# rdesc/autorally

Hardware: AMD Instinct MI355X
Metric: trajectory rollouts/s per MPPI solve (higher is better)
Workload: dtype f32

## Files before the change

### autorally_amd/csrc/abi_solve.hip

```cpp
#include "abi_internal.hpp"

using namespace mppi;
using namespace mppi_abi;

namespace mppi_abi {

std::mutex g_batch_mu;
hipStream_t g_batch_stream[64] = {};
hipStream_t batch_stream(int device)
{
  if (device < 0 || device >= 64) return nullptr;
  std::lock_guard<std::mutex> lk(g_batch_mu);
  if (!g_batch_stream[device] &&
      hipStreamCreateWithFlags(&g_batch_stream[device], hipStreamNonBlocking) != hipSuccess)
    g_batch_stream[device] = nullptr;
  return g_batch_stream[device];
}

void fill_cost_args(const mppi_handle *h, CostArgs &c)
{
  const mppi_cost_params &p = h->cost;
  c.desired_speed = p.desired_speed;
  c.speed_coeff = p.speed_coeff;
  c.track_coeff = p.track_coeff;
// ... 388 lines not shown
  if (rc) return rc;
  const bool timed = h->timing && (h->timing_count++ % (unsigned)h->timing_every) == 0;
  const bool explicit_noise = h->explicit_iters > 0;
  const size_t slot_sz = (size_t)K * T * 2;
  h->seq = next_seq(h);
  for (int it = 0; it < iters; it++) {
    Events *ev = timed ? &h->ev[it] : nullptr;
    if (ev) HIPCHK(h, hipEventRecord(ev->e[0], h->stream));
    const bool inline_noise = !explicit_noise && !h->prefetch_valid && has_noise_wave(h);
    float *noise = h->d_noise + (size_t)(explicit_noise ? it : 0) * slot_sz;
    if (!explicit_noise && !inline_noise) {
      rc = acquire_noise(h, &noise);
      if (rc) return rc;
    } else if (inline_noise) {
      noise = h->d_gen[h->gen_cur];
    }
    h->v_buf = noise;
    if (ev) HIPCHK(h, hipEventRecord(ev->e[1], h->stream));
    RolloutArgs a;
    fill_rollout_args(h, state, noise, a);
    rc = tag_min_cost(h, a, h->stream);
    if (rc) return rc;
    if (inline_noise) use_inline_noise(h, a);
#ifdef MPPI_HOSTPROF
    HP(1, hp_t0);
    const auto hp_t1 = std::chrono::steady_clock::now();
#endif
    if (ev) { tl_kernel_start = ev->e[4]; tl_kernel_stop = ev->e[5]; }
    rc = launch_rollout(h, a);
    tl_kernel_start = tl_kernel_stop = nullptr;
    if (rc) return rc;
#ifdef MPPI_HOSTPROF
    HP(2, hp_t1);
    const auto hp_t2 = std::chrono::steady_clock::now();
#endif
    const bool prefetch = h->gen_async && iters == 1 && !explicit_noise && !has_noise_wave(h) && !h->prefetch_valid;
    if (prefetch) HIPCHK(h, hipEventRecord(h->ev_s1, h->stream));
    if (ev) HIPCHK(h, hipEventRecord(ev->e[2], h->stream));
    const bool last = (it == iters - 1);
    const bool want_slid = last && wants_slid_copy(h);
    next_tail_epoch(h);
    HIPCHK(h, launch_solve_tail(tail_launch(h, noise, last), h->stream));
    if (last) h->slid_valid = want_slid;
    if (h->capture) {
      float *c = h->d_cap + (size_t)it * (2 * (size_t)T + K);
      if (!last) HIPCHK(h, hipMemcpyAsync(c, h->d_in, sizeof(float) * 2 * (size_t)T, hipMemcpyDeviceToDevice, h->stream));
      HIPCHK(h, hipMemcpyAsync(c + 2 * (size_t)T, h->d_costs, sizeof(float) * (size_t)K, hipMemcpyDeviceToDevice, h->stream));
    }
    if (prefetch) {
      h->gen_time_now = timed;
      rc = prefetch_noise(h);
      h->gen_time_now = false;
      if (rc) return rc;
    }
#ifdef MPPI_HOSTPROF
    HP(3, hp_t2);
    hp_n += 1;
    if ((long)hp_n % 2000 == 0)
      fprintf(stderr, "hostprof n=%.0f: seen->enqueue %.2f us, entry->launch %.2f, rollout launch %.2f, tail launch %.2f, poll->smoothed %.2f\n",
              hp_n, hp_acc[0] / hp_n, hp_acc[1] / hp_n, hp_acc[2] / hp_n, hp_acc[3] / hp_n, hp_acc[4] / hp_n);
#endif
    if (ev) HIPCHK(h, hipEventRecord(ev->e[3], h->stream));
  }
  h->explicit_iters = 0;
  h->pending = true;
  h->pending_timed = timed;
  h->cap_valid = h->capture;
  h->cap_explicit = explicit_noise;
  return MPPI_OK;
}


static int arm_kind(const mppi_handle *h)
{
  if (!(h->d_gate != nullptr && wants_slid_copy(h) && h->cfg.num_iters == 1 && !h->timing && !h->capture &&
        h->explicit_iters == 0 && !h->basis && h->fault_wave == 0 && h->have_nn && h->have_map && h->have_cost && !h->timed_out))
    return 0;
  const Form f = form_of(h);
  if ((form_is_row(f) || f == Form::M44 || f == Form::Lds44) && has_noise_wave(h) && !h->prefetch_valid) return 1;
  if (f == Form::Multi4Tree && h->forced == Form::Auto && !has_noise_wave(h) && h->gen_async && gen_beside_rollout(h)) return 2;
  return 0;
}

static void write_gate_payload(mppi_handle *h, const float *state)
{
  unsigned *g = gate_host(h);
  const int T = h->T;
  memcpy(g + kGateUOffset, h->U.data(), sizeof(float) * 2 * (size_t)T);
  memcpy(g + gate_hist_offset(T), h->hist.data(), sizeof(float) * 4);
  for (int r = 0; r < kGateReplicas; r++) memcpy(g + 16 * r, state, sizeof(float) * kStateDim);
}

static void write_gate_word(mppi_handle *h, unsigned word)
{
  unsigned *g = gate_host(h);
  asm volatile("" ::: "memory");
  __builtin_ia32_sfence();
  for (int r = 0; r < kGateReplicas; r++) __atomic_store_n(g + 16 * r + 7, word, __ATOMIC_RELAXED);
  __builtin_ia32_sfence();
}

static unsigned arm_ticks(double max_wait_s) { return (unsigned)(max_wait_s * 1e8); }
static std::chrono::steady_clock::time_point arm_deadline(double max_wait_s)
{
  const double open_s = 0.9 * max_wait_s - 50e-6;
  return std::chrono::steady_clock::now() + std::chrono::nanoseconds((long long)((open_s > 0.0 ? open_s : 0.0) * 1e9));
}

static void armed_args(mppi_handle *h, float *noise, RolloutArgs &a, TailLaunch &l, double max_wait_s)
{
  static const float no_state[kStateDim] = {0, 0, 0, 0, 0, 0, 0};
  fill_rollout_args(h, no_state, noise, a);
  a.costs = h->d_costs_alt;
  a.U = reinterpret_cast<const float *>(gate_dev(h)) + kGateUOffset;
  a.gate = gate_dev(h);
  a.gate_seq = h->arm_seq;
  a.gate_ticks = arm_ticks(max_wait_s);
  l = tail_launch(h, noise, true);
  l.costs = h->d_costs_alt;
  l.w = h->d_w_alt;
  l.seq = h->arm_seq;
  l.hist = reinterpret_cast<const float *>(gate_dev(h)) + gate_hist_offset(h->T);
  l.U = h->d_in;
  l.hist_out = h->d_in + 2 * h->T;
  l.slid = h->d_in_buf[1 - h->in_cur];
}

static void mark_armed(mppi_handle *h, int kind, float *vbuf, hipStream_t stream, double max_wait_s, bool publish_only)
{
  h->armed = kind;
  h->arm_in = h->in_cur;
  h->arm_vbuf = vbuf;
  h->arm_stream = stream;
  h->arm_until = arm_deadline(max_wait_s);
  h->arm_n = 0;
  h->arm_publish_only = publish_only;
  h->u_dirty = true;
  h->slid_valid = false;
}

static int arm_handle(mppi_handle *h, int kind, hipStream_t stream, double max_wait_s, bool publish_only, bool mark,
                      RolloutArgs &a, TailLaunch &l)
{
  h->arm_seq = next_seq(h);
  h->gate_blk ^= 1;
  float *noise = h->d_gen[1 - h->gen_cur];
  if (kind == 2) {
    int rc = acquire_noise(h, &noise);
    if (rc) return rc;
  }
  if (mark) HIPCHK(h, hipEventRecord(h->ev_arm, stream));
  armed_args(h, noise, a, l, max_wait_s);
  int rc = tag_min_cost(h, a, stream);
  if (rc) return rc;
  l.min_cost_tag = h->min_cost_tag;
  if (publish_only) {
    l.no_device_copy = 1;
    l.slid = nullptr;
  }
  if (kind == 1) use_inline_noise(h, a);
  next_tail_epoch(h);
  l.epoch = h->tail_epoch;
  mark_armed(h, kind, noise, stream, max_wait_s, publish_only);
  return MPPI_OK;
}

static int arm_one(mppi_handle *h, double max_wait_s, bool publish_only, bool mark)
{
  const int kind = arm_kind(h);
  if (!kind) return fail(h, MPPI_ERR_UNSUPPORTED, "this handle's form / configuration has no gated form (mppi_arm)");
  OWN(h);
  RolloutArgs a;
  TailLaunch l;
  int rc = arm_handle(h, kind, h->stream, max_wait_s, publish_only, mark, a, l);
  if (rc) return rc;
  rc = launch_rollout(h, a);
  if (rc == MPPI_OK) {
    const hipError_t e = launch_solve_tail(l, h->stream);
    if (e != hipSuccess) rc = fail(h, MPPI_ERR_HIP, "armed tail launch", e);
  }
  if (rc) (void)solve_ahead_disarm(h);
  return rc;
}

static int disarm_one(mppi_handle *h)
{
  if (!h->armed) return MPPI_OK;
  const int kind = h->armed;
  h->armed = 0;
  h->arm_n = 0;
  write_gate_word(h, h->arm_seq | kGateCancel);
  h->seq_floor = h->arm_seq;
  h->u_dirty = true;
  h->slid_valid = false;
  h->order_stream = h->arm_stream;
  if (kind == 1) {
    h->rng_cur = 1 - h->rng_cur;
    return MPPI_OK;
  }
  HIPCHK(h, ensure_device(h->cfg.device));
  h->gen_cur = 1 - h->gen_cur;
  h->rng_cur = 1 - h->rng_cur;
  HIPCHK(h, hipEventRecord(h->ev_s1, h->arm_stream));
  HIPCHK(h, hipStreamWaitEvent(h->gstream, h->ev_s1, 0));
  int rc = launch_generator(h, h->d_gen[1 - h->gen_cur]);
  if (rc) return rc;
  h->prefetch_valid = true;
  return MPPI_OK;
}

int solve_ahead_disarm(mppi_handle *h)
{
  if (!h || !h->armed) return MPPI_OK;
  if (h->arm_n > 0) {
    mppi_handle *peers[kMaxBatch];
    const int n = h->arm_n;
    for (int i = 0; i < n; i++) peers[i] = h->arm_peers[i];
    int rc = MPPI_OK;
    for (int i = 0; i < n; i++) {
      const int r = disarm_one(peers[i]);
      if (r && !rc) rc = r;
    }
    return rc;
  }
  return disarm_one(h);
}

static bool arm_usable(const mppi_handle *h)
{
  if (std::chrono::steady_clock::now() >= h->arm_until) return false;
  const volatile unsigned *words = reinterpret_cast<const volatile unsigned *>(h->h_res);
  const unsigned s1 = __atomic_load_n(words + 1, __ATOMIC_ACQUIRE), s3 = __atomic_load_n(words + 4 * (h->T + 1) + 1, __ATOMIC_ACQUIRE);
  return s1 != h->arm_seq && s3 != h->arm_seq;
}

static int open_armed(mppi_handle *h, const float *state)
{
  const int kind = h->armed;
  h->armed = 0;
  h->arm_n = 0;
  h->seq = h->arm_seq;
  write_gate_payload(h, state);
  write_gate_word(h, h->seq);
  h->order_stream = h->arm_stream;
  std::swap(h->d_costs, h->d_costs_alt);
  std::swap(h->d_w, h->d_w_alt);
  h->v_buf = h->arm_vbuf;
  if (kind == 1) h->gen_cur = h->arm_vbuf == h->d_gen[0] ? 0 : 1;
  h->in_cur = h->arm_in;
  h->d_in = h->d_in_buf[h->in_cur];
  h->u_dirty = h->arm_publish_only;
  h->slid_valid = !h->arm_publish_only;
  if (kind == 2) {
    const int rc = prefetch_noise(h);
    if (rc) {
      h->pending = true;
      h->pending_armed = true;
      return rc;
    }
  }
  h->pending = true;
  h->pending_timed = false;
  h->pending_armed = true;
  h->explicit_iters = 0;
  return MPPI_OK;
}

static bool batch_together(mppi_handle *const *hs, int n);
static int arm_together(mppi_handle *const *hs, int n, double max_wait_s)
{
  mppi_handle *h0 = hs[0];
  if (!form_is_row(form_of(h0))) return fail(h0, MPPI_ERR_UNSUPPORTED, "the batched launch of this form has no gated form");
  for (int i = 0; i < n; i++)
    if (arm_kind(hs[i]) != 1) return fail(hs[i], MPPI_ERR_UNSUPPORTED, "this handle's configuration has no gated form (mppi_arm_batch)");
  HIPCHK(h0, ensure_device(h0->cfg.device));
  if (!h0->batch_s) h0->batch_s = batch_stream(h0->cfg.device);
  const hipStream_t S = h0->batch_s;
  if (!S) return fail(h0, MPPI_ERR_HIP, "no batch stream");
  for (int i = 0; i < n; i++)
    if (int rc = hand_over(hs[i], S)) return rc;
  QuadBatchArgs qb;
  TailLaunch tl[kMaxBatch];
  qb.n = n;
  for (int i = 0; i < n; i++)
    if (int rc = arm_handle(hs[i], 1, S, max_wait_s, false, true, qb.inst[i], tl[i])) return rc;
  for (int i = 0; i < n; i++) {
    hs[i]->arm_n = n;
    for (int q = 0; q < n; q++) hs[i]->arm_peers[q] = hs[q];
  }
  for (int i = n; i < kMaxBatch; i++) qb.inst[i] = qb.inst[0];
  hipError_t e = launch_rollout_row_batch(qb, form_of(h0) == Form::RowTree, S);
  if (e == hipSuccess) e = launch_solve_tail_batch(tl, n, S);
  if (e != hipSuccess) {
    const int rc = fail(h0, MPPI_ERR_HIP, "armed batched launch", e);
    (void)solve_ahead_disarm(h0);
    return rc;
  }
  return MPPI_OK;
}

static bool batch_together(mppi_handle *const *hs, int n)
{
  const mppi_handle *h0 = hs[0];
  bool together = n >= 2 && n <= kMaxBatch;
  int waves = 0;
  for (int i = 0; i < n && together; i++) {
    const mppi_handle *h = hs[i];
    const Form f = form_of(h);
    const bool form_ok = h->basis ? (h0->basis && f == Form::Bf3)
                                  : (!h0->basis && (f == Form::Quad || form_is_row(f)) && f == form_of(h0) &&
                                     h->hidden == h0->hidden && h->n_hidden == h0->n_hidden);
    CostArgs ci, c0;
    fill_cost_args(h, ci);
    fill_cost_args(h0, c0);
    together = form_ok && ci.affine == c0.affine && ci.need_control_cost == c0.need_control_cost &&
               h->cfg.device == h0->cfg.device && h->cfg.num_iters == h0->cfg.num_iters &&
               h->K <= 4096 && !h->timing && !h->capture && !h->prefetch_valid && h->have_nn && h->have_map && h->have_cost;
    waves += h->basis ? 3 * (h->K / 64) : 4 * (h->K / kRolloutsPerWave);
  }
  return together && waves <= h0->num_simds;
}

static bool armed_as_batch(mppi_handle *const *hs, int n)
{
  for (int i = 0; i < n; i++) {
    if (!hs[i]->armed || hs[i]->arm_n != n) return false;
// ... 386 lines not shown
```

### autorally_amd/csrc/group_roles.hpp

```cpp
#pragma once

#include "mppi_device.hpp"
#include "noise_device.hpp"

namespace mppi {

constexpr int kGRing = 16;
constexpr int kGCtlChunk = 4;

template <class SH>
struct GroupRoles {
  static constexpr int kPose = SH::NW, kCost = SH::NW + 1, kCtl = SH::NW + 2, kRng = SH::NW + 3;
  static constexpr int kWaves = SH::NW + 4;
  static_assert(kWaves <= (int)(sizeof(SH::fin) / sizeof(int)), "fin[]");
  static_assert(SH::kR == 16 || SH::kR == 8, "rollouts per group");
};
template <class SH>
__device__ __forceinline__ int group_j(int slot) { return slot & (SH::kR - 1); }
template <class SH>
__device__ __forceinline__ bool group_real(int slot) { return slot < SH::kR; }

template <class SH>
__device__ __forceinline__ int group_seq_min(SH &sh)
{
// ... 1 lines not shown
#pragma unroll
  for (int w = 1; w < SH::NW; w++) m = min(m, lds_peek(lds_addr(&sh.xseq[w][0])));
  return m;
}

struct MrgHalf {
  uint32_t s0, s1, s2;
};
__device__ __forceinline__ uint32_t fold_m(uint64_t x, uint32_t C, uint32_t m)
{
  x = (x >> 32) * C + (x & 0xffffffffULL);
  x = (x >> 32) * C + (x & 0xffffffffULL);
  x = (x >> 32) * C + (x & 0xffffffffULL);
  if (x >= m) x -= m;
  return (uint32_t)x;
}
template <class SH>
__device__ __forceinline__ MrgHalf group_rng_load(const RolloutArgs &a)
{
  const int lane = threadIdx.x & 63;
  const int j = group_j<SH>((lane >> 1) & 15), c = lane & 1;
  const int k = (int)blockIdx.x * SH::kR + j;
  const int K = a.K;
  MrgHalf g{0, 0, 0};
  if (a.inline_noise != 0 && lane < 2 * kRolloutsPerWave) {
    g.s0 = a.rng_in[(3 * c) * K + k]; g.s1 = a.rng_in[(3 * c + 1) * K + k]; g.s2 = a.rng_in[(3 * c + 2) * K + k];
  }
  return g;
}
template <class SH, bool PRE = false>
__device__ __forceinline__ void group_rng_wave(const RolloutArgs &a, SH &sh, const MrgHalf pre = MrgHalf{0, 0, 0})
{
  using R = GroupRoles<SH>;
  const int lane = threadIdx.x & 63;
  const int j = group_j<SH>((lane >> 1) & 15), c = lane & 1;
  const int k = (int)blockIdx.x * SH::kR + j;
  const int K = a.K, T = a.T;
  const bool active = lane < 2 * kRolloutsPerWave;
  const bool real = lane < 2 * SH::kR;
  int budget = spin_budget_init(a.spin_budget, T, a.fault_wave == R::kRng + 1);
  if (a.inline_noise != 0) {
    const uint32_t m = c ? (uint32_t)kM2 : (uint32_t)kM1, C = c ? kC2 : kC1;
    const uint32_t A = c ? (uint32_t)kA21 : (uint32_t)kA12, Bn = c ? (uint32_t)kA23N : (uint32_t)kA13N;
    MrgHalf g{0, 0, 0};
    if constexpr (PRE) {
      g = pre;
    } else if (active) {
      g.s0 = a.rng_in[(3 * c) * K + k]; g.s1 = a.rng_in[(3 * c + 1) * K + k]; g.s2 = a.rng_in[(3 * c + 2) * K + k];
    }
    const uint32_t a_ctl = lds_addr(&sh.ctl_pub[0]);
    const uint32_t a_mypub = lds_addr(&sh.rng_pub[lane]);
    int seen = 0;
    for (int t = 0; t < T; t++) {
      float2 e = make_float2(0.5f, 0.5f);
#ifdef MPPI_DIAG_NORNG
      e = make_float2(0.25f + 0.001f * (float)t, 0.5f);
#else
#pragma unroll
      for (int d = 0; d < 2; d++) {
        const uint32_t p = fold_m((uint64_t)A * (c ? g.s2 : g.s1) + (uint64_t)Bn * (m - g.s0), C, m);
        g.s0 = g.s1; g.s1 = g.s2; g.s2 = p;
        const uint32_t p2 = (uint32_t)__builtin_amdgcn_mov_dpp((int)p, 0xB1, 0xF, 0xF, false);
        uint32_t z = (p >= p2) ? p - p2 : p + (uint32_t)kM1 - p2;
        if (z == 0) z = (uint32_t)kM1;
        const float u = (float)z * 0x1p-32f;
        if (d == 0) e.x = u; else e.y = u;
      }
#endif
      const int need = t - kGRing + 1;
      while (seen < need && --budget > 0) {
        seen = lds_peek(a_ctl);
        if (seen < need) __builtin_amdgcn_s_sleep(2);
      }
      if (active && c == 0) *reinterpret_cast<float2 *>(&sh.eps[t & (kGRing - 1)][j][0]) = e;
      lds_publish(a_mypub, t + 1);
    }
    if (real) {
      a.rng_out[(3 * c) * K + k] = g.s0; a.rng_out[(3 * c + 1) * K + k] = g.s1; a.rng_out[(3 * c + 2) * K + k] = g.s2;
    }
  }
  spin_finish(budget, lds_addr(&sh.fail[0]), lds_addr(&sh.fin[R::kRng]));
}

template <class SH>
__device__ __forceinline__ void group_control_wave(const RolloutArgs &a, SH &sh, const uint32_t a_gate_open = 0)
{
  using R = GroupRoles<SH>;
  constexpr int NSW = SH::NSW;
  static_assert(kGCtlChunk == 4 && kGRing >= 2 * kGCtlChunk, "four steps per iteration, lanes 16 q + j");
  const int lane = threadIdx.x & 63;
  const int j = group_j<SH>(lane & 15), q = lane >> 4;
  const bool real = group_real<SH>(lane & 15);
  const int k = (int)blockIdx.x * SH::kR + j;
  const int K = a.K, T = a.T;
  const bool inl = a.inline_noise != 0;
  float2 *const noise = reinterpret_cast<float2 *>(a.noise);
  const float2 *const Useq = reinterpret_cast<const float2 *>(a.U);
  const bool noise_free_k = (k == 0);
  const bool pure_noise_k = (k >= a.k99);
  const uint32_t a_cd = lds_addr(&sh.cost_done[0]);
  const uint32_t a_mypub = lds_addr(&sh.ctl_pub[lane]);
  const uint32_t a_rng = lds_addr(&sh.rng_pub[0]);
  int budget = spin_budget_init(a.spin_budget, T, a.fault_wave == R::kCtl + 1);
  const bool gated = a_gate_open != 0;
  if (gated)
    while (lds_peek(a_gate_open) == 0 && --budget > 0) __builtin_amdgcn_s_sleep(1);
  int seen_x = 0, seen_c = 0, seen_r = 0;
  for (int t0 = 0, n = 1; t0 < T; t0 += n, n = kGCtlChunk) {
    const int t = t0 + q;
    const bool live = (t < T) & (q < n);
    const int tl = live ? t : T - 1;
    float2 Ut;
    if (gated) {
      const unsigned long long ub = __hip_atomic_load(reinterpret_cast<const unsigned long long *>(Useq + tl), __ATOMIC_RELAXED, __HIP_MEMORY_SCOPE_SYSTEM);
      Ut = make_float2(__uint_as_float((unsigned)ub), __uint_as_float((unsigned)(ub >> 32)));
    } else {
      Ut = Useq[tl];
    }
    float2 e = (live && !inl) ? noise[(size_t)tl * K + k] : make_float2(0.0f, 0.0f);
    const int tm = min(t0 + n, T) - 1;
    const int need_x = (tm >= kGRing) ? (tm - kGRing) * NSW + 1 : 0;
    const int need_c = tm - kGRing + 1;
    while ((seen_x < need_x || seen_c < need_c) && --budget > 0) {
      seen_x = group_seq_min(sh);
      seen_c = lds_peek(a_cd);
      if (seen_x < need_x || seen_c < need_c) __builtin_amdgcn_s_sleep(2);
    }
    if (inl) {
      while (seen_r < tm + 1 && --budget > 0) {
        seen_r = lds_peek(a_rng);
        if (seen_r < tm + 1) __builtin_amdgcn_s_sleep(1);
      }
#ifdef MPPI_DIAG_NOBM
      e = *reinterpret_cast<const float2 *>(&sh.eps[tl & (kGRing - 1)][j][0]);
#else
      e = box_muller(*reinterpret_cast<const float2 *>(&sh.eps[tl & (kGRing - 1)][j][0]));
#endif
    }
    if (live) {
      const bool nf = noise_free_k | (t < a.opt_delay);
      const float n0 = e.x * a.nu[0], n1 = e.y * a.nu[1];
      const float du0 = nf ? 0.0f : n0, du1 = nf ? 0.0f : n1;
      float u0 = nf ? Ut.x : (pure_noise_k ? n0 : Ut.x + n0);
      float u1 = nf ? Ut.y : (pure_noise_k ? n1 : Ut.y + n1);
      if (real) noise[(size_t)t * K + k] = make_float2(u0, u1);
      u0 = clampf(u0, a.u_lo[0], a.u_hi[0]);
      u1 = clampf(u1, a.u_lo[1], a.u_hi[1]);
      const int slot = t & (kGRing - 1);
      sh.ctl_b1[slot][j] = u0;
      sh.ctl_b1[slot][kRolloutsPerWave + j] = u1;
      *reinterpret_cast<float4 *>(&sh.ctl_rec[slot][j][0]) = make_float4(u0, u1, du0, du1);
    }
    lds_publish(a_mypub, tm + 1);
  }
  spin_finish(budget, lds_addr(&sh.fail[0]), lds_addr(&sh.fin[R::kCtl]));
}

template <class SH, bool AFFINE>
__device__ __forceinline__ void group_pose_wave(const RolloutArgs &a, SH &sh)
{
  using R = GroupRoles<SH>;
  constexpr int NSW = SH::NSW;
  static_assert(SH::kR == 16, "one step per iteration: 16-rollout groups only");
  const int lane = threadIdx.x & 63;
  const int j = lane & 15;
  const int T = a.T;
  const uint32_t a_seq0 = lds_addr(&sh.xseq[0][0]);
  const uint32_t a_cd = lds_addr(&sh.cost_done[0]);
  const uint32_t a_mypub = lds_addr(&sh.pose_pub[lane]);
  float x = a.state[0], y = a.state[1], yaw = a.state[2];
  int budget = spin_budget_init(a.spin_budget, T, a.fault_wave == R::kPose + 1), seen = 0, cdone = 0;
  float tf_p = 0.0f, tb_p = 0.0f;
  for (int t = 0; t <= T; t++) {
    float tf = 0.0f, tb = 0.0f;
    if (t < T) {
      const int need = t * NSW + 1;
      while (seen < need && --budget > 0) {
        seen = SH::kRecByAll ? group_seq_min(sh) : lds_peek(a_seq0);
        if (seen < need) __builtin_amdgcn_s_sleep(1);
      }
      const float4 r0 = *reinterpret_cast<const float4 *>(&sh.rec[t & (kGRing - 1)][j][0]);
      float spsi, cpsi;
#ifdef MPPI_DIAG_NOPOSE
      spsi = 0.0f; cpsi = 1.0f; tf = x; tb = y;
#else
      sincos_fast(yaw, spsi, cpsi);
      const float st[3] = {x, y, yaw};
      track_fetch<AFFINE>(a.cost, st, cpsi, spsi, tf, tb);
#endif
      const float sd0 = fmaf(cpsi, r0.y, -(spsi * r0.z));
      const float sd1 = fmaf(spsi, r0.y, cpsi * r0.z);
      const float sd2 = a.negate_yaw_der ? -r0.w : r0.w;
      x = fmaf(sd0, a.dt, x);
      y = fmaf(sd1, a.dt, y);
      yaw = fmaf(sd2, a.dt, yaw);
    }
    if (t > 0) {
      while (cdone < t - kGRing && --budget > 0) cdone = lds_peek(a_cd);
      if (lane < kRolloutsPerWave) *reinterpret_cast<float2 *>(&sh.tex[(t - 1) & (kGRing - 1)][lane][0]) = make_float2(tf_p, tb_p);
      lds_publish(a_mypub, t);
    }
    tf_p = tf; tb_p = tb;
  }
  spin_finish(budget, lds_addr(&sh.fail[0]), lds_addr(&sh.fin[R::kPose]));
}

template <int Q>
__device__ __forceinline__ float quad_bc(float v)
{
  return __int_as_float(__builtin_amdgcn_mov_dpp(__float_as_int(v), Q * 0x55, 0xF, 0xF, false));
}
__device__ __forceinline__ void quad_chain(float v, float d, float dt, int q, float &vq, float &v_out)
{
  const float v1 = fmaf(quad_bc<0>(d), dt, v);
  const float v2 = fmaf(quad_bc<1>(d), dt, v1);
  const float v3 = fmaf(quad_bc<2>(d), dt, v2);
  v_out = fmaf(quad_bc<3>(d), dt, v3);
  const float lo = (q == 0) ? v : v1, hi = (q == 2) ? v2 : v3;
  vq = (q < 2) ? lo : hi;
}
template <class SH, bool AFFINE>
__device__ __forceinline__ void group_pose_wave4(const RolloutArgs &a, SH &sh, const float x0, const float y0, const float yaw0,
                                                 const int budget_cut = 0);
template <class SH, bool AFFINE>
__device__ __forceinline__ void group_pose_wave4(const RolloutArgs &a, SH &sh)
{
  group_pose_wave4<SH, AFFINE>(a, sh, a.state[0], a.state[1], a.state[2]);
}
template <class SH, bool AFFINE>
__device__ __forceinline__ void group_pose_wave4(const RolloutArgs &a, SH &sh, const float x0, const float y0, const float yaw0,
                                                 const int budget_cut)
{
  using R = GroupRoles<SH>;
  constexpr int NSW = SH::NSW;
  static_assert(kRolloutsPerWave == 16 && kGRing >= 8, "lane = 4 j + q");
  const int lane = threadIdx.x & 63;
// ... 160 lines not shown
```

### autorally_amd/csrc/mppi_device.hpp

```cpp
#pragma once

#include <hip/hip_runtime.h>
#include <stdint.h>

namespace mppi {

constexpr int kStateDim = 7;
constexpr int kControlDim = 2;
constexpr int kNetIn = 6;
constexpr int kNetOut = 4;
constexpr int kRolloutsPerWave = 16;

struct CostArgs {
  float desired_speed, speed_coeff, track_coeff, max_slip_ang, slip_penalty, track_slop;
  float crash_coeff, steering_coeff, throttle_coeff, boundary_threshold;
  float crash_cost_discounted;
  int l1_cost;
  float r_c1[3], r_c2[3], trs[3];
  int affine;
  int need_control_cost;
  int map_w, map_h;
  const float *map;
};

struct RolloutArgs {
  float state[kStateDim];
  const float *U;
  float *noise;
  float *costs;
  const float *wpack;
  const double *inv_t;
  const uint32_t *rng_in;
  uint32_t *rng_out;
  int inline_noise;
  int K, T, opt_delay, k99;
  float nu[2], u_lo[2], u_hi[2], dt;
  int negate_yaw_der;
  int spin_budget, fault_wave;
  const unsigned *gate;
  unsigned gate_seq;
  unsigned gate_ticks;
  unsigned long long *min_cost;
  unsigned min_cost_tag;
  CostArgs cost;
};
constexpr int kGateReplicas = 8;
constexpr int kGateUOffset = 16 * kGateReplicas;
inline int gate_hist_offset(int T) { return kGateUOffset + 2 * T; }
inline size_t gate_block_floats(int T) { return (size_t)gate_hist_offset(T) + 4; }
constexpr unsigned kGateCancel = 0x80000000u;

constexpr int kMinCostLines = 8, kMinCostStride = 16;
__device__ __forceinline__ unsigned cost_order_bits(float x)
{
  const unsigned b = __float_as_uint(x);
  return b ^ ((b >> 31) ? 0xFFFFFFFFu : 0x80000000u);
}
__device__ __forceinline__ float cost_from_order_bits(unsigned o)
{
  return __uint_as_float(o ^ ((o >> 31) ? 0x80000000u : 0xFFFFFFFFu));
}
template <int CTRL>
__device__ __forceinline__ float wave_dpp(float v)
{
  return __int_as_float(__builtin_amdgcn_update_dpp(0, __float_as_int(v), CTRL, 0xF, 0xF, true));
}
template <bool MIN>
__device__ __forceinline__ float wave_reduce(float v)
{
#define MPPI_RED(A, B) (MIN ? fminf((A), (B)) : (A) + (B))
  v = MPPI_RED(v, wave_dpp<0xB1>(v));
  v = MPPI_RED(v, wave_dpp<0x4E>(v));
  v = MPPI_RED(v, wave_dpp<0x141>(v));
  v = MPPI_RED(v, wave_dpp<0x140>(v));
  const auto x = __builtin_amdgcn_permlane16_swap(__float_as_uint(v), __float_as_uint(v), false, false);
  v = MPPI_RED(__uint_as_float(x[0]), __uint_as_float(x[1]));
  const auto y = __builtin_amdgcn_permlane32_swap(__float_as_uint(v), __float_as_uint(v), false, false);
  v = MPPI_RED(__uint_as_float(y[0]), __uint_as_float(y[1]));
#undef MPPI_RED
  return v;
}
__device__ __forceinline__ void publish_min_cost(const RolloutArgs &a, const float mine)
{
  if (a.min_cost == nullptr) return;
  const float m = wave_reduce<true>((mine == mine) ? mine : INFINITY);
  if ((threadIdx.x & 63) == 0 && m < INFINITY) {
    const unsigned long long key = ((unsigned long long)(~a.min_cost_tag) << 32) | cost_order_bits(m);
    (void)__hip_atomic_fetch_min(a.min_cost + (blockIdx.x % kMinCostLines) * kMinCostStride, key, __ATOMIC_RELAXED, __HIP_MEMORY_SCOPE_AGENT);
  }
}
__device__ __forceinline__ bool load_min_cost(const unsigned long long *min_cost, const unsigned tag, float &beta)
{
  if (min_cost == nullptr) return false;
  unsigned long long k[kMinCostLines];
#pragma unroll
  for (int i = 0; i < kMinCostLines; i++) k[i] = __hip_atomic_load(min_cost + i * kMinCostStride, __ATOMIC_RELAXED, __HIP_MEMORY_SCOPE_AGENT);
  unsigned long long best = k[0];
#pragma unroll
  for (int i = 1; i < kMinCostLines; i++) best = (k[i] < best) ? k[i] : best;
  beta = cost_from_order_bits((unsigned)best);
  return (unsigned)(best >> 32) == ~tag;
}

constexpr int kMaxBatch = 4;
template <int NB>
struct QuadBatchArgsT {
  int n;
  RolloutArgs inst[NB];
};
using QuadBatchArgs = QuadBatchArgsT<kMaxBatch>;
template <int NB>
inline QuadBatchArgsT<NB> batch_args_prefix(const QuadBatchArgs &b)
{
  QuadBatchArgsT<NB> s;
  s.n = b.n;
  for (int i = 0; i < NB; i++) s.inst[i] = b.inst[i];
  return s;
}
static_assert(kMaxBatch == 4, "MPPI_BATCH_DISPATCH");
#define MPPI_BATCH_DISPATCH(NB, B, BODY)     \
  do {                                      \
    if constexpr ((NB) == 2) {              \
      if (blockIdx.y == 0) BODY((B).inst[0]); \
      else BODY((B).inst[1]);               \
    } else {                                \
      switch ((int)blockIdx.y) {            \
        case 0: BODY((B).inst[0]); break;   \
        case 1: BODY((B).inst[1]); break;   \
        case 2: BODY((B).inst[2]); break;   \
        default: BODY((B).inst[3]); break;  \
      }                                     \
    }                                       \
  } while (0)
// ... 105 lines not shown
  const float slip = -atanf(s5 / fabsf(s4));
  float stab = c.slip_penalty * (slip * slip);
  stab = (fabsf(slip) > c.max_slip_ang) ? stab + c.crash_coeff : stab;
  o.stabilizing_cost = (fabsf(s4) >= kMinSpeed) ? stab : 0.0f;
}

__device__ __forceinline__ float cost_terms_b(const CostArgs &c, const CostTerms &a, float tf, float tb,
                                              int &crash)
{
  float track_cost = (fabsf(tf) + fabsf(tb)) * 0.5f;
  track_cost = (fabsf(track_cost) < c.track_slop) ? 0.0f : c.track_coeff * track_cost;
  crash |= (int)(tf >= c.boundary_threshold) | (int)(tb >= c.boundary_threshold);
  const float crash_cost = (crash > 0) ? c.crash_cost_discounted : 0.0f;
  float cost = a.control_cost + a.speed_cost + crash_cost + track_cost + a.stabilizing_cost;
  cost = (cost >= kCostCapGt || cost != cost) ? kCostCap : cost;
  return cost;
}

template <bool CTRL_COST>
__device__ __forceinline__ float cost_finish(const CostArgs &c, const float nu[2], float s4, float s5,
                                             float tf, float tb, float u0, float u1, float du0,
                                             float du1, int &crash)
{
  CostTerms t;
  cost_terms_a<CTRL_COST>(c, nu, s4, s5, u0, u1, du0, du1, t);
  return cost_terms_b(c, t, tf, tb, crash);
}

__device__ __forceinline__ float running_mean(float J, float c, int t, double rt)
{
  const double d = (double)(c - J);
  const double td = (double)t;
  const double q0 = d * rt;
  const double e = fma(-q0, td, d);
  const double q = fma(e, rt, q0);
  return (float)((double)J + q);
}

constexpr int kSpinBudget = 1 << 22;

__device__ __forceinline__ uint32_t lds_addr(const void *p)
{
  return (uint32_t)(uintptr_t)(const __attribute__((address_space(3))) void *)p;
}
__device__ __forceinline__ void lds_publish(uint32_t addr, int v)
{
  asm volatile("ds_write_b32 %0, %1" ::"v"(addr), "v"(v) : "memory");
}
__device__ __forceinline__ void lds_put4(uint32_t addr, f32x4 v)
{
  asm volatile("ds_write_b128 %0, %1" ::"v"(addr), "v"(v) : "memory");
}
__device__ __forceinline__ int lds_peek(uint32_t addr)
{
  int v;
  asm volatile("ds_read_b32 %0, %1\n\ts_waitcnt lgkmcnt(0)" : "=&v"(v) : "v"(addr) : "memory");
  return __builtin_amdgcn_readfirstlane(v);
}
__device__ __forceinline__ float row_sel(int g, float s3, float s4, float s5, float s6)
{
  const float lo = (g == 0) ? s3 : s4;
  const float hi = (g == 2) ? s5 : s6;
  return (g < 2) ? lo : hi;
}

__device__ __forceinline__ int lds_peek_lanes(uint32_t addr)
{
  int v;
  asm volatile("ds_read_b32 %0, %1\n\ts_waitcnt lgkmcnt(0)" : "=&v"(v) : "v"(addr) : "memory");
  return v;
}

__device__ __forceinline__ int spin_budget_init(int spin_budget, int T, bool inject_fault)
{
  if (inject_fault) return 0;
  return (spin_budget > 0 ? spin_budget : kSpinBudget) + 64 * T;
}
__device__ __forceinline__ void spin_finish(int budget, uint32_t a_fail, uint32_t a_fin)
{
  if (budget <= 0) lds_publish(a_fail, 1);
  lds_publish(a_fin, 1);
}

template <class SH>
__device__ __forceinline__ int group_gate_wait(const RolloutArgs &a, SH &sh)
{
  const int lane = threadIdx.x & 63;
  const unsigned *blk = a.gate + (size_t)((int)blockIdx.x % kGateReplicas) * 16;
  const unsigned long long t0 = __builtin_amdgcn_s_memrealtime();
  unsigned v = 0;
  for (;;) {
    v = __hip_atomic_load(blk + 7, __ATOMIC_RELAXED, __HIP_MEMORY_SCOPE_SYSTEM);
    if ((v & ~kGateCancel) == a.gate_seq) break;
    if (__builtin_amdgcn_s_memrealtime() - t0 > (unsigned long long)a.gate_ticks) { v = kGateCancel; break; }
    __builtin_amdgcn_s_sleep(2);
  }
  asm volatile("" ::: "memory");
  const float sv = __uint_as_float(__hip_atomic_load(blk + (lane & 7), __ATOMIC_RELAXED, __HIP_MEMORY_SCOPE_SYSTEM));
  if (lane < 7) sh.gstate[lane] = sv;
  lds_publish(lds_addr(&sh.gate_open[0]), 1);
  return (v & kGateCancel) ? 1 : 0;
}


}
```

### autorally_amd/csrc/rollout_row.hip

```cpp
#include "group_roles.hpp"
#include "mppi_kernels.hpp"

namespace mppi {

#ifdef MPPI_ROW_STAMPS
__device__ unsigned long long g_row_stamps[16];
#define RSTAMP(i)                                                                                         \
  do {                                                                                                    \
    if (blockIdx.x == 0 && (threadIdx.x & 63) == 0) {                                                     \
      unsigned long long t__;                                                                             \
      asm volatile("s_memtime %0\n\ts_waitcnt lgkmcnt(0)" : "=s"(t__)::"memory");                           \
      g_row_stamps[i] = t__;                                                                              \
    }                                                                                                     \
  } while (0)
#else
#define RSTAMP(i) do { } while (0)
#endif

template <int H>
struct RowShared {
  static constexpr int NW = 4;
  static constexpr int NSW = 1;
  static constexpr bool kRecByAll = true;
  static constexpr int kR = 16;
  int xseq[NW][64];
  float rec[kGRing][kRolloutsPerWave][4];
  int cost_done[64];
  float ctl_b1[kGRing][64];
  float ctl_rec[kGRing][kRolloutsPerWave][4];
  int ctl_pub[64];
  float tex[kGRing][kRolloutsPerWave][2];
  int pose_pub[64];
  float eps[kGRing][kRolloutsPerWave][2];
  int rng_pub[64];
  int fail[4];
  int fin[8];
  float gstate[8];
  int gate_open[8];
  float dump[NW][64 * 2 + (kGRing - 1) * kRolloutsPerWave * 4];
};

template <int H, bool TREE>
struct RowWeights {
  f32x2 w1[kNetIn], w2[H], w3[TREE ? 4 : H];
  f32x2 b1s, b2s, b3;
};

constexpr int kRowPackEntries = 40;
template <int H, bool TREE>
__device__ __forceinline__ void row_load(const float *rowpack, int p, RowWeights<H, TREE> &W)
{
  static_assert(H == 32, "entry layout of pack_row_weights");
  const float4 *pk = reinterpret_cast<const float4 *>(rowpack) + p;
#pragma unroll
  for (int i = 0; i < 3; i++) {
    const float4 v = pk[i * 16];
    W.w1[2 * i] = f32x2{v.x, v.y};
    W.w1[2 * i + 1] = f32x2{v.z, v.w};
  }
#pragma unroll
  for (int i = 0; i < H / 2; i++) {
    const float4 v = pk[(3 + i) * 16];
    W.w2[2 * i] = f32x2{v.x, v.y};
    W.w2[2 * i + 1] = f32x2{v.z, v.w};
    if constexpr (!TREE) {
      const float4 u = pk[(3 + H / 2 + i) * 16];
      W.w3[2 * i] = f32x2{u.x, u.y};
      W.w3[2 * i + 1] = f32x2{u.z, u.w};
    }
  }
  const float4 b = pk[35 * 16];
  W.b1s = f32x2{b.x, b.y};
  W.b2s = f32x2{b.z, b.w};
  if constexpr (TREE) {
    const float4 u = pk[37 * 16], v = pk[38 * 16], c = pk[39 * 16];
    W.w3[0] = f32x2{u.x, u.y};
    W.w3[1] = f32x2{u.z, u.w};
    W.w3[2] = f32x2{v.x, v.y};
    W.w3[3] = f32x2{v.z, v.w};
    W.b3 = f32x2{c.x, c.y};
  } else {
    const float4 c = pk[36 * 16];
    W.b3 = f32x2{c.x, c.y};
  }
}

template <int Q>
__device__ __forceinline__ float row_bc(float a)
{
  return __int_as_float(__builtin_amdgcn_mov_dpp(__float_as_int(a), 0x150 + Q, 0xF, 0xF, false));
}
template <int Q>
__device__ __forceinline__ f32x2 row_bc2(f32x2 a)
{
  return __builtin_bit_cast(f32x2, (long long)__builtin_amdgcn_mov_dpp(__builtin_bit_cast(long long, a), 0x150 + Q, 0xF, 0xF, false));
}
template <int Q>
__device__ __forceinline__ void row_dot_step(f32x2 &z, f32x2 &b, const f32x2 *w, f32x2 a)
{
  z = __builtin_elementwise_fma(w[2 * Q], f32x2{b.x, b.x}, z);
// ... 102 lines not shown

  const uint32_t a_myseq = lds_addr(&sh.xseq[w][lane]);
  typedef const volatile int __attribute__((address_space(3))) *lds_int_p;
  typedef const volatile f32x2 __attribute__((address_space(3))) *lds_f2_p;
  const lds_int_p p_pub = (lds_int_p)&sh.ctl_pub[0];
  uint32_t a_u0 = lds_addr(&sh.ctl_rec[0][jr][0]);
  asm volatile("" : "+v"(a_u0));
  const lds_f2_p p_u = (lds_f2_p)a_u0;
  const uint32_t a_rec0 = TREE ? (((p & 3) == 0) ? lds_addr(&sh.rec[0][jr][p >> 2]) : lds_addr(&sh.dump[w][2 * lane]))
                               : ((p < 2) ? lds_addr(&sh.rec[0][jr][2 * p]) : lds_addr(&sh.dump[w][2 * lane]));
  constexpr uint32_t kRecStride = sizeof(float) * kRolloutsPerWave * 4;

  int budget = spin_budget_init(a.spin_budget, T, a.fault_wave == w + 1);
  f32x2 sp;
  if constexpr (GATED) {
    const uint32_t a_go = lds_addr(&sh.gate_open[0]);
    while (lds_peek(a_go) == 0 && --budget > 0) __builtin_amdgcn_s_sleep(1);
    const volatile float *gs = sh.gstate;
    sp = TREE ? f32x2{gs[3 + (p >> 2)], 0.0f} : odd ? f32x2{gs[5], gs[6]} : f32x2{gs[3], gs[4]};
  } else {
    sp = TREE ? f32x2{a.state[3 + (p >> 2)], 0.0f} : odd ? f32x2{a.state[5], a.state[6]} : f32x2{a.state[3], a.state[4]};
  }
  if (w == 0) RSTAMP(2);
  int cp = 0;
  while ((cp = __builtin_amdgcn_readfirstlane(*p_pub)) < 1 && --budget > 0) __builtin_amdgcn_s_sleep(1);
  if (w == 0) RSTAMP(3);
  lds_f2_p pu = p_u;
  f32x2 un = pu[0];
  asm volatile("" : "+v"(un));

  const int NS = T - 1;
  for (int t0 = 0; t0 < NS; t0 += 4) {
    const uint32_t a_rec = a_rec0 + (uint32_t)(t0 & (kGRing - 1)) * kRecStride;
    row_step<H, TREE, 0>(a, W, sp, un, t0, a_rec, a_myseq, p_pub, pu, p_u, cp, budget);
    if (t0 + 1 >= NS) break;
    row_step<H, TREE, 1>(a, W, sp, un, t0, a_rec, a_myseq, p_pub, pu, p_u, cp, budget);
    if (t0 + 2 >= NS) break;
    row_step<H, TREE, 2>(a, W, sp, un, t0, a_rec, a_myseq, p_pub, pu, p_u, cp, budget);
    if (t0 + 3 >= NS) break;
    row_step<H, TREE, 3>(a, W, sp, un, t0, a_rec, a_myseq, p_pub, pu, p_u, cp, budget);
  }
  if (w == 0) RSTAMP(4);
  {
    const int t = T - 1;
    if constexpr (TREE) asm volatile("ds_write_b32 %0, %1" ::"v"(a_rec0 + (uint32_t)(t & (kGRing - 1)) * kRecStride), "v"(sp.x) : "memory");
    else asm volatile("ds_write_b64 %0, %1" ::"v"(a_rec0 + (uint32_t)(t & (kGRing - 1)) * kRecStride), "v"(sp) : "memory");
    lds_publish(a_myseq, t + 1);
  }
  spin_finish(budget, lds_addr(&sh.fail[0]), lds_addr(&sh.fin[w]));
}

template <int H, bool AFFINE, bool CTRL, bool TREE, bool GATED = false>
__device__ __forceinline__ void row_group(const RolloutArgs &a, RowShared<H> &sh)
{
  using SH = RowShared<H>;
  using R = GroupRoles<SH>;
  const int lane = threadIdx.x & 63;
  const int role = __builtin_amdgcn_readfirstlane(threadIdx.x >> 6);
  if (role == 0) RSTAMP(0);
  MrgHalf g0{0, 0, 0};
  if (role == R::kRng) g0 = group_rng_load<SH>(a);
  if (role == 0) {
#pragma unroll
    for (int w = 0; w < 4; w++) sh.xseq[w][lane] = 0;
    sh.cost_done[lane] = 0;
    sh.ctl_pub[lane] = 0;
    sh.pose_pub[lane] = 0;
    sh.rng_pub[lane] = 0;
    sh.fail[lane & 3] = 0;
    sh.fin[lane & 7] = 0;
    sh.gate_open[lane & 7] = 0;
  }
  __syncthreads();
  if (role == 0) RSTAMP(1);
#ifdef MPPI_ROW_RIDER_PRIO
  if (role >= 4) __builtin_amdgcn_s_setprio(MPPI_ROW_RIDER_PRIO);
#endif
  if (role < 4) row_dynamics<H, TREE, GATED>(a, sh, role);
  else if (role == R::kCost) { group_cost_wave4<SH, CTRL>(a, sh); RSTAMP(5); }
  else if (role == R::kCtl) { group_control_wave(a, sh, GATED ? lds_addr(&sh.gate_open[0]) : 0u); RSTAMP(6); }
  else if (role == R::kPose) {
    if constexpr (GATED) {
      const int shut = group_gate_wait(a, sh);
      const volatile float *gs = sh.gstate;
      const float x0 = gs[0], y0 = gs[1], yaw0 = gs[2];
      group_pose_wave4<SH, AFFINE>(a, sh, x0, y0, yaw0, shut);
    } else {
      group_pose_wave4<SH, AFFINE>(a, sh);
    }
    RSTAMP(7);
  }
  else { group_rng_wave<SH, true>(a, sh, g0); RSTAMP(8); }
}

template <int H, bool AFFINE, bool CTRL, bool TREE>
__global__ __launch_bounds__(512) void rollout_row_kernel(const RolloutArgs a)
{
  __shared__ __attribute__((aligned(16))) RowShared<H> sh;
  row_group<H, AFFINE, CTRL, TREE>(a, sh);
}
template <int H, bool AFFINE, bool CTRL, bool TREE>
__global__ __launch_bounds__(512) void rollout_row_gated_kernel(const RolloutArgs a)
{
  __shared__ __attribute__((aligned(16))) RowShared<H> sh;
  row_group<H, AFFINE, CTRL, TREE, true>(a, sh);
}

template <int H, bool AFFINE, bool CTRL, bool TREE, int NB>
__global__ __launch_bounds__(512) void rollout_row_batch_kernel(const QuadBatchArgsT<NB> b)
{
  __shared__ __attribute__((aligned(16))) RowShared<H> sh;
#define MPPI_ROW_BODY(A)                                                                                   \
  do {                                                                                                     \
    if ((int)blockIdx.x >= (A).K / kRolloutsPerWave) return;      \
    row_group<H, AFFINE, CTRL, TREE>((A), sh);                                                             \
  } while (0)
  MPPI_BATCH_DISPATCH(NB, b, MPPI_ROW_BODY);
#undef MPPI_ROW_BODY
}

template <int H, bool AFFINE, bool CTRL, bool TREE, int NB>
__global__ __launch_bounds__(512) void rollout_row_batch_gated_kernel(const QuadBatchArgsT<NB> b)
{
  __shared__ __attribute__((aligned(16))) RowShared<H> sh;
#define MPPI_ROW_BODY(A)                                                                                   \
  do {                                                                                                     \
    if ((int)blockIdx.x >= (A).K / kRolloutsPerWave) return;      \
    row_group<H, AFFINE, CTRL, TREE, true>((A), sh);                                                       \
  } while (0)
  MPPI_BATCH_DISPATCH(NB, b, MPPI_ROW_BODY);
#undef MPPI_ROW_BODY
}

bool row_variant_supported(int hidden, int n_hidden) { return hidden == 32 && n_hidden == 2; }
int row_pack_floats() { return kRowPackEntries * 16 * 4; }

#define MPPI_ROW_DISPATCH(LAUNCH, KERN, TREE, ...)                                                            \
  do {                                                                                                        \
    if (affine && !ctrl) LAUNCH((KERN<32, true, false, TREE>), __VA_ARGS__);                                  \
    else if (affine && ctrl) LAUNCH((KERN<32, true, true, TREE>), __VA_ARGS__);                               \
    else if (!affine && !ctrl) LAUNCH((KERN<32, false, false, TREE>), __VA_ARGS__);                           \
    else LAUNCH((KERN<32, false, true, TREE>), __VA_ARGS__);                                                  \
  } while (0)
#define MPPI_ROW_BATCH_DISPATCH(KERN, TREE, NB, ...)                                                                            \
  do {                                                                                                                          \
    if (affine && !ctrl) hipLaunchKernelGGL((KERN<32, true, false, TREE, NB>), __VA_ARGS__);                                    \
    else if (affine && ctrl) hipLaunchKernelGGL((KERN<32, true, true, TREE, NB>), __VA_ARGS__);                                 \
    else if (!affine && !ctrl) hipLaunchKernelGGL((KERN<32, false, false, TREE, NB>), __VA_ARGS__);                             \
    else hipLaunchKernelGGL((KERN<32, false, true, TREE, NB>), __VA_ARGS__);                                                    \
  } while (0)

hipError_t launch_rollout_row_batch(const QuadBatchArgs &b, bool tree, hipStream_t stream)
{
  if (b.n < 1 || b.n > kMaxBatch) return hipErrorInvalidValue;
  bool affine = true, ctrl = false;
  int gmax = 0;
  const bool gated = b.inst[0].gate != nullptr;
  for (int i = 0; i < b.n; i++) {
    if ((b.inst[i].gate != nullptr) != gated) return hipErrorInvalidValue;
    affine = affine && b.inst[i].cost.affine != 0;
    ctrl = ctrl || b.inst[i].cost.need_control_cost != 0;
    gmax = b.inst[i].K / kRolloutsPerWave > gmax ? b.inst[i].K / kRolloutsPerWave : gmax;
  }
  const dim3 grid(gmax, b.n), block(512);
  if (b.n <= 2) {
    const QuadBatchArgsT<2> b2 = batch_args_prefix<2>(b);
// ... 45 lines not shown
```

Before: 107.1 million.

## Pack gate state and sequence into one cache line; prefetch control noise before gate

The host now writes each gate replica as a single 64-byte line in which every state float is paired with the sequence number. The device can then check that a whole line is fresh with one ballot over eight 64-bit loads, where before it polled a flag word and then reread the state. Cancel becomes a single 64-bit store into the control granule. The control wave no longer waits on the LDS gate flag before doing anything. It draws and scales its first two noise chunks while it polls the gate control granule directly, then preloads the first U values. This removes latency from the armed solve's critical path after the host opens the gate, at the cost of more complex gate protocol logic and extra stamp instrumentation.

```diff
diff --git a/autorally_amd/csrc/abi_solve.hip b/autorally_amd/csrc/abi_solve.hip
--- a/autorally_amd/csrc/abi_solve.hip
+++ b/autorally_amd/csrc/abi_solve.hip
@@ -494,21 +494,38 @@
   return 0;
 }
 
-static void write_gate_payload(mppi_handle *h, const float *state)
+static void write_gate_payload(mppi_handle *h)
 {
   unsigned *g = gate_host(h);
   const int T = h->T;
   memcpy(g + kGateUOffset, h->U.data(), sizeof(float) * 2 * (size_t)T);
   memcpy(g + gate_hist_offset(T), h->hist.data(), sizeof(float) * 4);
-  for (int r = 0; r < kGateReplicas; r++) memcpy(g + 16 * r, state, sizeof(float) * kStateDim);
-}
-
-static void write_gate_word(mppi_handle *h, unsigned word)
+}
+
+static void write_gate_lines(mppi_handle *h, const float *state, unsigned seq)
 {
   unsigned *g = gate_host(h);
+  alignas(64) unsigned line[16];
+  for (int i = 0; i < kStateDim; i++) {
+    memcpy(&line[2 * i], &state[i], sizeof(float));
+    line[2 * i + 1] = seq;
+  }
+  line[2 * kGateCtlGranule] = 0;
+  line[2 * kGateCtlGranule + 1] = seq;
   asm volatile("" ::: "memory");
   __builtin_ia32_sfence();
-  for (int r = 0; r < kGateReplicas; r++) __atomic_store_n(g + 16 * r + 7, word, __ATOMIC_RELAXED);
+  for (int r = 0; r < kGateReplicas; r++) memcpy(__builtin_assume_aligned(g + 16 * r, 64), line, sizeof(line));
+  asm volatile("" ::: "memory");
+  __builtin_ia32_sfence();
+}
+
+static void write_gate_cancel(mppi_handle *h, unsigned seq)
+{
+  unsigned long long *g = reinterpret_cast<unsigned long long *>(gate_host(h));
+  const unsigned long long v = ((unsigned long long)seq << 32) | kGateCancel;
+  asm volatile("" ::: "memory");
+  __builtin_ia32_sfence();
+  for (int r = 0; r < kGateReplicas; r++) __atomic_store_n(g + 8 * r + kGateCtlGranule, v, __ATOMIC_RELAXED);
   __builtin_ia32_sfence();
 }
 
@@ -601,7 +618,7 @@
   const int kind = h->armed;
   h->armed = 0;
   h->arm_n = 0;
-  write_gate_word(h, h->arm_seq | kGateCancel);
+  write_gate_cancel(h, h->arm_seq);
   h->seq_floor = h->arm_seq;
   h->u_dirty = true;
   h->slid_valid = false;
@@ -652,8 +669,8 @@
   h->armed = 0;
   h->arm_n = 0;
   h->seq = h->arm_seq;
-  write_gate_payload(h, state);
-  write_gate_word(h, h->seq);
+  write_gate_payload(h);
+  write_gate_lines(h, state, h->seq);
   h->order_stream = h->arm_stream;
   std::swap(h->d_costs, h->d_costs_alt);
   std::swap(h->d_w, h->d_w_alt);
diff --git a/autorally_amd/csrc/group_roles.hpp b/autorally_amd/csrc/group_roles.hpp
--- a/autorally_amd/csrc/group_roles.hpp
+++ b/autorally_amd/csrc/group_roles.hpp
@@ -107,6 +107,9 @@
   spin_finish(budget, lds_addr(&sh.fail[0]), lds_addr(&sh.fin[R::kRng]));
 }
 
+#ifndef MPPI_GROUP_STAMP
+#define MPPI_GROUP_STAMP(i) do { } while (0)
+#endif
 template <class SH>
 __device__ __forceinline__ void group_control_wave(const RolloutArgs &a, SH &sh, const uint32_t a_gate_open = 0)
 {
@@ -128,20 +131,49 @@
   const uint32_t a_rng = lds_addr(&sh.rng_pub[0]);
   int budget = spin_budget_init(a.spin_budget, T, a.fault_wave == R::kCtl + 1);
   const bool gated = a_gate_open != 0;
-  if (gated)
-    while (lds_peek(a_gate_open) == 0 && --budget > 0) __builtin_amdgcn_s_sleep(1);
   int seen_x = 0, seen_c = 0, seen_r = 0;
-  for (int t0 = 0, n = 1; t0 < T; t0 += n, n = kGCtlChunk) {
+  auto draw = [&](int tl, int tm) __attribute__((always_inline)) {
+    while (seen_r < tm + 1 && --budget > 0) {
+      seen_r = lds_peek(a_rng);
+      if (seen_r < tm + 1) __builtin_amdgcn_s_sleep(1);
+    }
+#ifdef MPPI_DIAG_NOBM
+    return *reinterpret_cast<const float2 *>(&sh.eps[tl & (kGRing - 1)][j][0]);
+#else
+    return box_muller(*reinterpret_cast<const float2 *>(&sh.eps[tl & (kGRing - 1)][j][0]));
+#endif
+  };
+  const int tl1 = min(1 + q, T - 1);
+  float2 n_pre0 = make_float2(0.0f, 0.0f), n_pre1 = n_pre0, U_pre0 = n_pre0, U_pre1 = n_pre0;
+  if (gated) {
+    if (inl) {
+      const float2 e0 = draw(0, 0);
+      n_pre0 = make_float2(e0.x * a.nu[0], e0.y * a.nu[1]);
+      if (T > 1) {
+        const float2 e1 = draw(tl1, min(1 + kGCtlChunk, T) - 1);
+        n_pre1 = make_float2(e1.x * a.nu[0], e1.y * a.nu[1]);
+      }
+    }
+    const unsigned long long *line = gate_line(a);
+    for (;;) {
+      const int v = __builtin_amdgcn_readfirstlane(gate_ctl_peek(a, line));
+      if (v > 0) break;
+      if (v < 0 || lds_peek(a_gate_open) == kGateShut) { budget = 0; break; }
+      if (--budget <= 0) break;
+      __builtin_amdgcn_s_sleep(2);
+    }
+    U_pre0 = gate_load_u(Useq);
+    U_pre1 = gate_load_u(Useq + tl1);
+  }
+  for (int t0 = 0, n = 1, it = 0; t0 < T; t0 += n, n = kGCtlChunk, it++) {
     const int t = t0 + q;
     const bool live = (t < T) & (q < n);
     const int tl = live ? t : T - 1;
+    const bool pre = gated & (it < 2);
     float2 Ut;
-    if (gated) {
-      const unsigned long long ub = __hip_atomic_load(reinterpret_cast<const unsigned long long *>(Useq + tl), __ATOMIC_RELAXED, __HIP_MEMORY_SCOPE_SYSTEM);
-      Ut = make_float2(__uint_as_float((unsigned)ub), __uint_as_float((unsigned)(ub >> 32)));
-    } else {
-      Ut = Useq[tl];
-    }
+    if (pre) Ut = (it == 0) ? U_pre0 : U_pre1;
+    else if (gated) Ut = gate_load_u(Useq + tl);
+    else Ut = Useq[tl];
     float2 e = (live && !inl) ? noise[(size_t)tl * K + k] : make_float2(0.0f, 0.0f);
     const int tm = min(t0 + n, T) - 1;
     const int need_x = (tm >= kGRing) ? (tm - kGRing) * NSW + 1 : 0;
@@ -151,20 +183,16 @@
       seen_c = lds_peek(a_cd);
       if (seen_x < need_x || seen_c < need_c) __builtin_amdgcn_s_sleep(2);
     }
-    if (inl) {
-      while (seen_r < tm + 1 && --budget > 0) {
-        seen_r = lds_peek(a_rng);
-        if (seen_r < tm + 1) __builtin_amdgcn_s_sleep(1);
-      }
-#ifdef MPPI_DIAG_NOBM
-      e = *reinterpret_cast<const float2 *>(&sh.eps[tl & (kGRing - 1)][j][0]);
-#else
-      e = box_muller(*reinterpret_cast<const float2 *>(&sh.eps[tl & (kGRing - 1)][j][0]));
-#endif
+    float2 nn;
+    if (pre && inl) {
+      nn = (it == 0) ? n_pre0 : n_pre1;
+    } else {
+      if (inl) e = draw(tl, tm);
+      nn = make_float2(e.x * a.nu[0], e.y * a.nu[1]);
     }
     if (live) {
       const bool nf = noise_free_k | (t < a.opt_delay);
-      const float n0 = e.x * a.nu[0], n1 = e.y * a.nu[1];
+      const float n0 = nn.x, n1 = nn.y;
       const float du0 = nf ? 0.0f : n0, du1 = nf ? 0.0f : n1;
       float u0 = nf ? Ut.x : (pure_noise_k ? n0 : Ut.x + n0);
       float u1 = nf ? Ut.y : (pure_noise_k ? n1 : Ut.y + n1);
@@ -177,6 +205,7 @@
       *reinterpret_cast<float4 *>(&sh.ctl_rec[slot][j][0]) = make_float4(u0, u1, du0, du1);
     }
     lds_publish(a_mypub, tm + 1);
+    if (gated && it < 2) { if (it == 0) MPPI_GROUP_STAMP(10); else MPPI_GROUP_STAMP(11); }
   }
   spin_finish(budget, lds_addr(&sh.fail[0]), lds_addr(&sh.fin[R::kCtl]));
 }
diff --git a/autorally_amd/csrc/mppi_device.hpp b/autorally_amd/csrc/mppi_device.hpp
--- a/autorally_amd/csrc/mppi_device.hpp
+++ b/autorally_amd/csrc/mppi_device.hpp
@@ -49,6 +49,8 @@
 inline int gate_hist_offset(int T) { return kGateUOffset + 2 * T; }
 inline size_t gate_block_floats(int T) { return (size_t)gate_hist_offset(T) + 4; }
 constexpr unsigned kGateCancel = 0x80000000u;
+constexpr int kGateCtlGranule = 7;
+constexpr int kGateOpened = 1, kGateShut = 2;
 
 constexpr int kMinCostLines = 8, kMinCostStride = 16;
 __device__ __forceinline__ unsigned cost_order_bits(float x)
@@ -320,25 +322,42 @@
   lds_publish(a_fin, 1);
 }
 
+__device__ __forceinline__ const unsigned long long *gate_line(const RolloutArgs &a)
+{
+  return reinterpret_cast<const unsigned long long *>(a.gate) + (size_t)((int)blockIdx.x % kGateReplicas) * 8;
+}
 template <class SH>
 __device__ __forceinline__ int group_gate_wait(const RolloutArgs &a, SH &sh)
 {
   const int lane = threadIdx.x & 63;
-  const unsigned *blk = a.gate + (size_t)((int)blockIdx.x % kGateReplicas) * 16;
+  const unsigned long long *gran = gate_line(a) + (lane & 7);
   const unsigned long long t0 = __builtin_amdgcn_s_memrealtime();
-  unsigned v = 0;
+  unsigned long long g;
+  int shut = 0;
   for (;;) {
-    v = __hip_atomic_load(blk + 7, __ATOMIC_RELAXED, __HIP_MEMORY_SCOPE_SYSTEM);
-    if ((v & ~kGateCancel) == a.gate_seq) break;
-    if (__builtin_amdgcn_s_memrealtime() - t0 > (unsigned long long)a.gate_ticks) { v = kGateCancel; break; }
+    g = __hip_atomic_load(gran, __ATOMIC_RELAXED, __HIP_MEMORY_SCOPE_SYSTEM);
+    const unsigned hit = (unsigned)__builtin_amdgcn_ballot_w64((unsigned)(g >> 32) == a.gate_seq) & 0xffu;
+    const unsigned ctl = (unsigned)__builtin_amdgcn_readlane((int)(unsigned)g, kGateCtlGranule);
+    if ((hit >> kGateCtlGranule) != 0 && (ctl & kGateCancel) != 0) { shut = 1; break; }
+    if (hit == 0xffu) break;
+    if (__builtin_amdgcn_s_memrealtime() - t0 > (unsigned long long)a.gate_ticks) { shut = 1; break; }
     __builtin_amdgcn_s_sleep(2);
   }
-  asm volatile("" ::: "memory");
-  const float sv = __uint_as_float(__hip_atomic_load(blk + (lane & 7), __ATOMIC_RELAXED, __HIP_MEMORY_SCOPE_SYSTEM));
-  if (lane < 7) sh.gstate[lane] = sv;
-  lds_publish(lds_addr(&sh.gate_open[0]), 1);
-  return (v & kGateCancel) ? 1 : 0;
-}
-
-
-}
+  if (lane < 7) sh.gstate[lane] = __uint_as_float((unsigned)g);
+  lds_publish(lds_addr(&sh.gate_open[0]), shut ? kGateShut : kGateOpened);
+  return shut;
+}
+__device__ __forceinline__ int gate_ctl_peek(const RolloutArgs &a, const unsigned long long *line)
+{
+  const unsigned long long g = __hip_atomic_load(line + kGateCtlGranule, __ATOMIC_RELAXED, __HIP_MEMORY_SCOPE_SYSTEM);
+  if ((unsigned)(g >> 32) != a.gate_seq) return 0;
+  return ((unsigned)g & kGateCancel) ? -1 : 1;
+}
+__device__ __forceinline__ float2 gate_load_u(const float2 *p)
+{
+  const unsigned long long ub = __hip_atomic_load(reinterpret_cast<const unsigned long long *>(p), __ATOMIC_RELAXED, __HIP_MEMORY_SCOPE_SYSTEM);
+  return make_float2(__uint_as_float((unsigned)ub), __uint_as_float((unsigned)(ub >> 32)));
+}
+
+
+}
diff --git a/autorally_amd/csrc/rollout_row.hip b/autorally_amd/csrc/rollout_row.hip
--- a/autorally_amd/csrc/rollout_row.hip
+++ b/autorally_amd/csrc/rollout_row.hip
@@ -1,8 +1,6 @@
-#include "group_roles.hpp"
-#include "mppi_kernels.hpp"
+#include "mppi_device.hpp"
 
 namespace mppi {
-
 #ifdef MPPI_ROW_STAMPS
 __device__ unsigned long long g_row_stamps[16];
 #define RSTAMP(i)                                                                                         \
@@ -13,9 +11,16 @@
       g_row_stamps[i] = t__;                                                                              \
     }                                                                                                     \
   } while (0)
+#define MPPI_GROUP_STAMP(i) RSTAMP(i)
 #else
 #define RSTAMP(i) do { } while (0)
 #endif
+}
+
+#include "group_roles.hpp"
+#include "mppi_kernels.hpp"
+
+namespace mppi {
 
 template <int H>
 struct RowShared {
@@ -284,6 +289,7 @@
   else if (role == R::kPose) {
     if constexpr (GATED) {
       const int shut = group_gate_wait(a, sh);
+      RSTAMP(9);
       const volatile float *gs = sh.gstate;
       const float x0 = gs[0], y0 = gs[1], yaw0 = gs[2];
       group_pose_wave4<SH, AFFINE>(a, sh, x0, y0, yaw0, shut);
```

Result: slower. 102.9 million (-3.9%).
